# paritybit-ai/XFL

Measured on AMD Instinct MI355X. Metric: 2048-bit Paillier encrypts/s (device-resident), higher is better.
Workload: dtype u32; 1 GPU; DJN private-key (CRT) encrypt, obfuscated, precision 7, 1000000 float64 plaintexts/GPU resident in HBM; key_bits=2048, elements_per_gpu=1000000, fixed_base_window_bits=23, fixed_base_window_split=False, parallelism=shard1, table_bytes=193273528320

## Files before the change

### xfl_amd/csrc/keyconst.hpp

```cpp
#pragma once
#include <algorithm>
#include <cstdint>
#include <stdexcept>
#include <utility>
#include <vector>

#include "hostbn.hpp"
#include "keydev.hpp"
#include "rns_layout.hpp"

namespace xhe {

struct ModSpec {
  int S, W;
  int S4() const { return (S + 3) & ~3; }
  BigU R() const { return pow2((size_t)W * S); }
};

struct KeySpec {
  int K;
  bool priv, djn;
  ModSpec mp2, mp2L, mp2X;
  ModSpec mp;
  ModSpec mn2, mn2X;
// ... 205 lines not shown
using PairF = const uint2* KeyDev::*;
using ModF = ModDev KeyDev::*;
using IntF = int KeyDev::*;

struct Dst {
  RowF w = nullptr;
  PairF d = nullptr;
  ModF m = nullptr;
  const uint32_t* ModDev::*mw = nullptr;
  size_t* off = nullptr;
  Dst(RowF f) : w(f) {}
  Dst(PairF f) : d(f) {}
  Dst(ModF mod, const uint32_t* ModDev::*f) : m(mod), mw(f) {}
  Dst(size_t* o) : off(o) {}
};

struct KeyImage {
  std::vector<uint32_t> words;
  KeyDev kd{};
  int rand_bits = 0, rand_words = 0;
  size_t hM_n2 = 0, hM_p2[2] = {0, 0};
  std::vector<uint32_t> hinvM_p[2];

  void put(const std::vector<uint32_t>& v, Dst dst, size_t min_words = 0) {
    const size_t off = words.size();
    const size_t len = (std::max(v.size(), min_words) + 3) & ~(size_t)3;
    words.resize(off + len, 0u);
    std::copy(v.begin(), v.end(), words.begin() + off);
    if (dst.off) *dst.off = off;
    else binds.push_back({dst, off});
  }
  void put_limbs(const BigU& x, const ModSpec& s, Dst dst) { put(x.to_limbs(s.W, s.S), dst, s.S4()); }
  void put_words(const BigU& x, int nw, Dst dst) {
    std::vector<uint32_t> v(nw);
    x.to_words(v.data(), nw);
    put(v, dst);
  }
  void put_mod(const BigU& M, const ModSpec& s, ModF m, int npow = 0) {
    const BigU R1 = mod(s.R(), M), R2 = mulmod(R1, R1, M), R3 = mulmod(R2, R1, M);
    put_limbs(M, s, {m, &ModDev::N});
    put_limbs(R1, s, {m, &ModDev::R1});
    put_limbs(R2, s, {m, &ModDev::R2});
    put_limbs(R3, s, {m, &ModDev::R3});
    (kd.*m).n0inv = mont_ninv(M.word(0), s.W);
    if (npow <= 0) return;
    std::vector<uint32_t> rows((size_t)npow * s.S4(), 0u);
    BigU x = mod(BigU(1), M);
    for (int j = 0; j < npow; ++j) {
      const std::vector<uint32_t> l = x.to_limbs(s.W, s.S);
      std::copy(l.begin(), l.end(), rows.begin() + (size_t)j * s.S4());
      x = mulmod(x, R1, M);
    }
    put(rows, {m, &ModDev::Rpow});
  }

  KeyDev bind(const uint32_t* base) const {
    KeyDev r = kd;
    for (const Binding& b : binds) {
      const uint32_t* p = base + b.off;
      if (b.dst.w) r.*b.dst.w = p;
      else if (b.dst.d) r.*b.dst.d = reinterpret_cast<const uint2*>(p);
      else (r.*b.dst.m).*b.dst.mw = p;
    }
    return r;
  }

 private:
  struct Binding {
    Dst dst;
    size_t off;
  };
  std::vector<Binding> binds;
};

namespace pq {
constexpr ModF m2[2] = {&KeyDev::p2, &KeyDev::q2}, m2L[2] = {&KeyDev::p2L, &KeyDev::q2L},
               m2X[2] = {&KeyDev::p2X, &KeyDev::q2X}, m1[2] = {&KeyDev::p, &KeyDev::q},
               dm[2] = {&KeyDev::dp, &KeyDev::dq};
constexpr RowF nprime[2] = {&KeyDev::p2_nprime, &KeyDev::q2_nprime}, rns[2] = {&KeyDev::rns_p, &KeyDev::rns_q},
               nR2[2] = {&KeyDev::nR2_p2, &KeyDev::nR2_q2}, nR2L[2] = {&KeyDev::nR2_p2L, &KeyDev::nR2_q2L},
               nR[2] = {&KeyDev::nR_p2, &KeyDev::nR_q2}, R1C[2] = {&KeyDev::R1C_p2X, &KeyDev::R1C_q2X},
               nR2C[2] = {&KeyDev::nR2C_p2X, &KeyDev::nR2C_q2X}, m1_words[2] = {&KeyDev::pm1_words, &KeyDev::qm1_words},
               inv_lim[2] = {&KeyDev::pinv_lim, &KeyDev::qinv_lim}, hR[2] = {&KeyDev::hpR, &KeyDev::hqR},
               topc[2] = {&KeyDev::topc_p, &KeyDev::topc_q}, e_words[2] = {&KeyDev::ep_words, &KeyDev::eq_words},
               x_kn2[2] = {&KeyDev::x_kn2_p, &KeyDev::x_kn2_q}, x_rmn[2] = {&KeyDev::x_rmn_p, &KeyDev::x_rmn_q},
               x_topc[2] = {&KeyDev::x_topc_p, &KeyDev::x_topc_q}, x_fold[2] = {&KeyDev::x_fold_p, &KeyDev::x_fold_q},
               x_hpR[2] = {&KeyDev::x_hpR_p, &KeyDev::x_hpR_q};
constexpr PairF x_dwt[2] = {&KeyDev::x_dwt_p, &KeyDev::x_dwt_q}, x_dw[2] = {&KeyDev::x_dw_p, &KeyDev::x_dw_q};
constexpr IntF m1_bits[2] = {&KeyDev::pm1_bits, &KeyDev::qm1_bits}, e_bits[2] = {&KeyDev::ep_bits, &KeyDev::eq_bits};
}

struct Prime {
  BigU X, Y, X2, n, h;
};

struct DigitMod {
  const BigU& M;
  ModSpec s;
  BigU R, RM, Rinv;
  DigitMod(const BigU& M_, const ModSpec& s_) : M(M_), s(s_), R(s_.R()), RM(mod(R, M_)), Rinv(modinv(RM, M_)) {}
};

inline std::vector<uint32_t> digit_pairs(const DigitMod& d, const BigU& Xw) {
  const BigU e = mulmod(mod(Xw, d.M), d.Rinv, d.M);
  BigU Q;
  divmod(add(Xw, mul(d.R, sub(d.M, e))), d.M, &Q, nullptr);
  const BigU f = submod(mod(Q, d.M), d.RM, d.M);
  const std::vector<uint32_t> el = e.to_limbs(d.s.W, d.s.S), fl = f.to_limbs(d.s.W, d.s.S);
  std::vector<uint32_t> v(2 * (size_t)d.s.S);
  for (int i = 0; i < d.s.S; ++i) {
    v[2 * i] = el[i];
    v[2 * i + 1] = fl[i];
  }
  return v;
}

inline std::vector<uint32_t> mask_plus_e(const BigU& M, const BigU& RM, const ModSpec& s) {
  std::vector<uint32_t> v = submod(BigU(1), RM, M).to_limbs(s.W, s.S);
  for (auto& x : v) x += (1u << s.W) - 1u;
  return v;
}

inline void digit_modulus(KeyImage& im, const DigitMod& d, const BigU& M2, ModF m, RowF kn2, RowF rmn) {
  im.put_mod(d.M, d.s, m);
  BigU c;
  divmod(sub(add(d.R, d.M), BigU(1)), d.M, &c, nullptr);
  im.put_limbs(mul(c, M2), ModSpec{2 * d.s.S, d.s.W}, kn2);
  im.put_limbs(sub(d.R, d.M), d.s, rmn);
}

inline void n2_constants(KeyImage& im, const KeySpec& s, const BigU& n, const BigU& n2, const BigU* h_pub) {
  im.put_words(n, s.nw(), &KeyDev::n_words);
  im.put_words(n2, s.n2w(), &KeyDev::n2_words);
  BigU maxpos;
  divmod(n, BigU(3), &maxpos, nullptr);
  im.put_words(maxpos, s.nw(), &KeyDev::maxpos);
  im.put_words(sub(n, maxpos), s.nw(), &KeyDev::minneg);
  im.put_limbs(n, s.mp2, &KeyDev::n_lim);
  im.put_mod(n2, s.mn2, &KeyDev::n2, kRpowRows);
  im.put_mod(n2, s.mn2X, &KeyDev::n2X, kRpowRows);
  if (s.K == 2048) {
    BigU mu;
    divmod(pow2((size_t)s.bar.W * 2 * s.bar.S), n2, &mu, nullptr);
    im.put_limbs(mu, ModSpec{s.bar.S + 1, s.bar.W}, &KeyDev::n2_mu);
  }
  if (s.K == 2048) {
    const ModSpec& sw = s.wave;
    const BigU Rw = sw.R();
    im.put_limbs(n2, sw, &KeyDev::n2w_N);
    im.put_limbs(sub(Rw, modinv(n2, Rw)), sw, &KeyDev::n2w_np);
    const BigU Rwn = mod(Rw, n2), Rw2 = mulmod(Rwn, Rwn, n2);
    im.put_limbs(mulmod(Rw2, modinv(mod(s.mn2X.R(), n2), n2), n2), sw, &KeyDev::n2w_C);
    im.put_limbs(Rw2, sw, &KeyDev::n2w_R2);
  }
  im.put_mod(n, s.mp2L, &KeyDev::nL);
  im.put_limbs(n2, ModSpec{2 * s.mp2L.S, s.mp2L.W}, &KeyDev::n2_limL);
  const BigU Rn2 = mod(s.mn2.R(), n2);
  im.put_limbs(mulmod(n, mulmod(Rn2, Rn2, n2), n2), s.mn2, &KeyDev::nR2_n2);
  if (h_pub) im.put_limbs(mulmod(mod(*h_pub, n2), Rn2, n2), s.mn2, &im.hM_n2);
}

inline void ndigit_constants(KeyImage& im, const KeySpec& s, const BigU& n, const BigU& n2) {
  const DigitMod d(n, s.nd);
  digit_modulus(im, d, n2, &KeyDev::nd, &KeyDev::nd_kn2, &KeyDev::nd_rmn);
  const BigU Rn2 = mod(d.R, n2), R2 = mulmod(Rn2, Rn2, n2), R4 = mulmod(R2, R2, n2);
  im.put(digit_pairs(d, R2), &KeyDev::nd_d1);
  im.put(digit_pairs(d, R4), &KeyDev::nd_dw);
  im.put(digit_pairs(d, mulmod(R4, modinv(mod(s.mn2.R(), n2), n2), n2)), &KeyDev::nd_dwt);
  im.put(mask_plus_e(n, d.RM, d.s), &KeyDev::nd_topc);
}

inline void prime2_constants(KeyImage& im, const KeySpec& s, const Prime (&pr)[2], const BigU* h, int nwin) {
  const ModSpec &s2 = s.mp2, &sL = s.mp2L, &sx = s.mp2X;
  const BigU &p2 = pr[0].X2, &q2 = pr[1].X2;
  im.put_mod(p2, s2, &KeyDev::p2);
  for (int i = 0; i < 2; ++i) im.put_mod(pr[i].X2, sL, pq::m2L[i]);
  for (int i = 0; i < 2; ++i) im.put_mod(pr[i].X2, sx, pq::m2X[i]);
  im.put_mod(q2, s2, &KeyDev::q2);
  const BigU R = s2.R();
  if (s.K == 2048) {
    for (int i = 0; i < 2; ++i) im.put_limbs(sub(R, modinv(pr[i].X2, R)), s2, pq::nprime[i]);
    im.put(rnsh::bases().shared, &KeyDev::rns);
    for (int i = 0; i < 2; ++i) im.put(rnsh::prime_block(pr[i].X), pq::rns[i]);
  }
  const BigU Rm[2] = {mod(R, p2), mod(R, q2)};
  for (int i = 0; i < 2; ++i)
    im.put_limbs(mulmod(pr[i].n, mulmod(Rm[i], Rm[i], pr[i].X2), pr[i].X2), s2, pq::nR2[i]);
  const BigU RL = sL.R();
  for (int i = 0; i < 2; ++i) {
    const BigU RLm = mod(RL, pr[i].X2);
    im.put_limbs(mulmod(pr[i].n, mulmod(RLm, RLm, pr[i].X2), pr[i].X2), sL, pq::nR2L[i]);
  }
  for (int i = 0; i < 2; ++i) im.put_limbs(mulmod(pr[i].n, Rm[i], pr[i].X2), s2, pq::nR[i]);
  im.put_limbs(mulmod(modinv(q2, p2), Rm[0], p2), s2, &KeyDev::q2invR_p2);
  im.put_limbs(q2, s2, &KeyDev::q2_lim);
  im.put_limbs(shl(p2, 2), s2, &KeyDev::p2x4_lim);
  if (!s.djn) return;
  for (int i = 0; i < 2; ++i)
    im.put_limbs(mulmod(mod(*h, pr[i].X2), Rm[i], pr[i].X2), s2, &im.hM_p2[i]);
  const BigU Rx = sx.R(), Cexp = pow2((size_t)(sx.S - s2.S) * s2.W * nwin);
  for (int i = 0; i < 2; ++i) {
    const BigU& X2 = pr[i].X2;
    const BigU RxP = mod(Rx, X2), CR = mulmod(mod(Cexp, X2), RxP, X2);
    im.put_limbs(CR, sx, pq::R1C[i]);
    im.put_limbs(mulmod(pr[i].n, mulmod(CR, RxP, X2), X2), sx, pq::nR2C[i]);
  }
}

inline void decrypt_constants(KeyImage& im, const KeySpec& s, const BigU& n, Prime (&pr)[2]) {
  const ModSpec& s1 = s.mp;
  const BigU T = s1.R();
  for (int i = 0; i < 2; ++i) im.put_mod(pr[i].X, s1, pq::m1[i]);
  for (int i = 0; i < 2; ++i) {
    const BigU m1 = sub(pr[i].X, BigU(1));
    im.kd.*pq::m1_bits[i] = (int)m1.bits();
    im.put_words(m1, s.nw() / 2 + 1, pq::m1_words[i]);
  }
  for (int i = 0; i < 2; ++i) im.put_limbs(modinv(pr[i].X, T), s1, pq::inv_lim[i]);
  BigU Tm[2];
  for (int i = 0; i < 2; ++i) {
    const BigU& X = pr[i].X;
    const BigU x = mod(add(BigU(1), mul(sub(X, BigU(1)), n)), pr[i].X2);
    BigU L;
    divmod(sub(x, BigU(1)), X, &L, nullptr);
    pr[i].h = modinv(L, X);
    Tm[i] = mod(T, X);
  }
  for (int i = 0; i < 2; ++i) im.put_limbs(mulmod(pr[i].h, Tm[i], pr[i].X), s1, pq::hR[i]);
  im.put_limbs(mulmod(modinv(pr[1].X, pr[0].X), Tm[0], pr[0].X), s1, &KeyDev::qinvpR);
  im.put_limbs(pr[1].X, s1, &KeyDev::q_lim);
  if (s.K == 2048)
    for (int i = 0; i < 2; ++i) im.put(mask_plus_e(pr[i].X, mod(s.pmd.R(), pr[i].X), s.pmd), pq::topc[i]);
}

inline void pdigit_constants(KeyImage& im, const KeySpec& s, const Prime& pr, int i) {
  const BigU &X = pr.X, &X2 = pr.X2;
  const DigitMod d(X, s.pd);
  digit_modulus(im, d, X2, pq::dm[i], pq::x_kn2[i], pq::x_rmn[i]);
  im.put(mask_plus_e(X, d.RM, d.s), pq::x_topc[i]);
  im.put_limbs(mulmod(mod(pr.Y, X), mulmod(mulmod(d.RM, d.RM, X), d.RM, X), X), d.s, pq::x_fold[i]);
  const BigU Rx2 = mod(d.R, X2), R2 = mulmod(Rx2, Rx2, X2), R4 = mulmod(R2, R2, X2);
  im.put(digit_pairs(d, mulmod(R4, modinv(mod(s.mp2.R(), X2), X2), X2)), pq::x_dwt[i]);
  im.put(digit_pairs(d, R4), pq::x_dw[i]);
  im.put_limbs(mulmod(pr.h, d.RM, X), d.s, pq::x_hpR[i]);
}

inline void exponent_constants(KeyImage& im, const KeySpec& s, const BigU& n, const Prime (&pr)[2]) {
  im.put_limbs(shl(pr[0].X, 1), s.mp, &KeyDev::p2x_lim);
  im.put_limbs(pr[0].X, s.mp, &KeyDev::p_lim);
  for (int i = 0; i < 2; ++i) {
    const BigU e = mod(n, mul(pr[i].X, sub(pr[i].X, BigU(1))));
    im.kd.*pq::e_bits[i] = (int)e.bits();
    im.put_words(e, s.nw(), pq::e_words[i]);
  }
}

inline std::vector<uint32_t> inverse_base_limbs(const ModSpec& s, const BigU& h, const BigU& P) {
  std::vector<uint32_t> v = mulmod(modinv(mod(h, P), P), mod(s.R(), P), P).to_limbs(s.W, s.S);
  v.resize((size_t)s.S4(), 0u);
  return v;
}

inline KeyImage derive_key_constants(const KeySpec& s, const BigU& n, const BigU* p, const BigU* q, const BigU* h) {
  KeyImage im;
  KeyDev& kd = im.kd;
  kd.K = s.K;
  kd.nw = s.nw();
  kd.n2w = s.n2w();
  kd.priv = s.priv;
  kd.djn = s.djn;
  kd.n_bits = (int)n.bits();
  im.rand_bits = s.djn ? (int)(n.bits() / 2) : (int)n.bits();
  im.rand_words = (im.rand_bits + 31) / 32;
  if (s.djn) {
    kd.win = s.win;
    win_layout(im.rand_bits, s.win, s.priv && s.split, &kd.nwin, &kd.nhi);
  }
  const BigU n2 = mul(n, n);
  n2_constants(im, s, n, n2, s.djn && !s.priv ? h : nullptr);
  if (s.K == 2048) {
    kd.ndig = 1;
    ndigit_constants(im, s, n, n2);
  }
  if (!s.priv) return im;
  Prime pr[2] = {{*p, *q, mul(*p, *p), {}, {}}, {*q, *p, mul(*q, *q), {}, {}}};
  for (Prime& x : pr) x.n = mod(n, x.X2);
  prime2_constants(im, s, pr, h, kd.nwin);
  decrypt_constants(im, s, n, pr);
  if (s.K != 2048) {
    kd.pmdx_dec = 1;
    for (int i = 0; i < 2; ++i) pdigit_constants(im, s, pr[i], i);
  }
  exponent_constants(im, s, n, pr);
  if (s.K == 2048 && s.djn)
    for (int i = 0; i < 2; ++i) im.hinvM_p[i] = inverse_base_limbs(s.pmd, *h, pr[i].X);
  return im;
}

}
```

### xfl_amd/csrc/keydev.hpp

```cpp
#pragma once
#include <cstdint>

#include <hip/hip_vector_types.h>

namespace xhe {

struct ModDev {
  const uint32_t* N;
  const uint32_t* R1;
  const uint32_t* R2;
  const uint32_t* R3;
  uint32_t n0inv;
  const uint32_t* Rpow;
};

constexpr int kRawChunk = 32;
constexpr int kRpowRows = kRawChunk + 2;

struct KeyDev {
  int K, nw, n2w;
  int priv, djn;
  const uint32_t* n_words;
  const uint32_t* n2_words;
  const uint32_t* maxpos;
  const uint32_t* minneg;
  const uint32_t* n_lim;
  ModDev n2;
  const uint32_t* nR2_n2;
  const uint32_t* tab_n2;
  const uint32_t* ep_words;
  const uint32_t* eq_words;
  int ep_bits, eq_bits, n_bits;
  ModDev p2, q2;
  ModDev p2L, q2L;
  ModDev p2X, q2X;
  ModDev n2X;
  const uint32_t* nR2_p2;
  const uint32_t *nR_p2, *nR_q2;
  const uint32_t *nR2C_p2X, *nR2C_q2X;
  const uint32_t *R1C_p2X, *R1C_q2X;
  const uint32_t* nR2_q2;
  const uint32_t* nR2_p2L;
  const uint32_t* nR2_q2L;
  const uint32_t* q2invR_p2;
  const uint32_t* q2_lim;
  const uint32_t* p2x4_lim;
  const uint32_t* tab_p2;
  const uint32_t* tab_q2;
  int64_t tab_rs;
  int win, nwin, nhi;
  ModDev p, q;
  const uint32_t* pm1_words;
  const uint32_t* qm1_words;
  int pm1_bits, qm1_bits;
  const uint32_t* pinv_lim;
  const uint32_t* qinv_lim;
  const uint32_t* hpR;
  const uint32_t* hqR;
  const uint32_t* qinvpR;
  const uint32_t* q_lim;
  const uint32_t* p2x_lim;
  const uint32_t* p_lim;
  int pmd;
  const uint32_t *topc_p, *topc_q;
  int ndig;
  ModDev nd;
  const uint32_t *nd_kn2, *nd_rmn, *nd_topc;
  const uint2 *nd_dw, *nd_d1;
  const uint2* nd_dwt;
  int pub_nd;
  int pmdx;
  ModDev dp, dq;
  const uint32_t *x_kn2_p, *x_kn2_q, *x_rmn_p, *x_rmn_q, *x_topc_p, *x_topc_q, *x_fold_p, *x_fold_q;
  const uint2 *x_dwt_p, *x_dwt_q;
  int pmdx_dec;
  const uint2 *x_dw_p, *x_dw_q;
  const uint32_t *x_hpR_p, *x_hpR_q;
  const uint32_t *p2_nprime, *q2_nprime;
  const uint32_t *rns, *rns_p, *rns_q;
  const uint32_t *n2w_N, *n2w_np, *n2w_C, *n2w_R2;
  const uint32_t* n2_mu;
  ModDev nL;
  const uint32_t* n2_limL;
};

}
```

### xfl_amd/csrc/pdigit_dev.hpp

```cpp
#pragma once
#include "bn_dev.hpp"

namespace xhe {

struct PmdLdsQ {
  const uint32_t* q;
  XHE_DEV uint4 load4(int i) const { return *reinterpret_cast<const uint4*>(q + (i >> 2) * 256); }
};

template <int K_>
struct PMD {
  static constexpr int K = K_, W = 28, BL = 6;
  static constexpr int NQ = (2 * K + 3) / 4;
  static constexpr uint32_t MASK = (1u << W) - 1u;
  static_assert((K - 1) % BL == 0, "positions 1..K-1 in blocks of 6");
  static_assert((double)(3 * K + 2) * (double)(1ull << 57) < 18446744073709551616.0, "accumulator bound");

  uint32_t p[K];
  uint32_t n0inv;

  XHE_DEV void init(const uint32_t* __restrict__ P, uint32_t ninv) {
#pragma unroll
    for (int j = 0; j < K; ++j) p[j] = __builtin_amdgcn_readfirstlane(P[j]);
    n0inv = ninv;
// ... 191 lines not shown
      "v_mad_u64_u32 %10, vcc, %16, %33, %10\n\t"
      "v_mad_u64_u32 %11, vcc, %16, %34, %11"
        : "+v"(T1[j - 1]), "+v"(T1[j]), "+v"(T1[j + 1]), "+v"(T1[j + 2]), "+v"(T1[j + 3]), "+v"(T1[j + 4]),
          "+v"(T2[j - 1]), "+v"(T2[j]), "+v"(T2[j + 1]), "+v"(T2[j + 2]), "+v"(T2[j + 3]), "+v"(T2[j + 4])
        : "v"(T1[j + 5]), "v"(T2[j + 5]), "v"(e), "v"(m1), "v"(m2), "v"(a[j]), "v"(a[j + 1]), "v"(a[j + 2]),
          "v"(a[j + 3]), "v"(a[j + 4]), "v"(a[j + 5]), "v"(c[j]), "v"(c[j + 1]), "v"(c[j + 2]), "v"(c[j + 3]),
          "v"(c[j + 4]), "v"(c[j + 5]), "s"(p[j]), "s"(p[j + 1]), "s"(p[j + 2]), "s"(p[j + 3]), "s"(p[j + 4]),
          "s"(p[j + 5])
        : "vcc");
  }

  XHE_DEV void step_row(uint64_t (&T1)[K], uint64_t (&T2)[K], const uint32_t (&a)[K], const uint32_t (&c)[K],
                        uint32_t e, uint32_t en, uint32_t& m1, uint32_t& m2, uint64_t& x1, uint64_t& x2,
                        uint32_t topc) const {
    uint64_t x1n = 0, x2n = 0;
    uint32_t t1 = 0, t2 = 0, m1n = 0, m2n = 0;
    asm("v_mad_u64_u32 %0, vcc, %2, %4, %0\n\t"
        "v_mad_u64_u32 %1, vcc, %3, %4, %1"
        : "+v"(x1), "+v"(x2)
        : "v"(m1), "v"(m2), "s"(p[0])
        : "vcc");
#pragma unroll
    for (int b = 0; b < (K - 1) / BL; ++b) {
      const int j = 1 + BL * b;
      blk12_row(T1, T2, a, c, e, m1, m2, j);
      if (b == 0) {
        T1[0] += x1 >> W;
        T2[0] += x2 >> W;
        asm volatile("" : "+v"(T1[0]), "+v"(T2[0]));
      } else if (b == 1) {
        asm("v_mad_u64_u32 %0, vcc, %2, %3, %5\n\t"
            "v_mad_u64_u32 %1, vcc, %2, %4, %6"
            : "=&v"(x1n), "=&v"(x2n)
            : "v"(en), "v"(a[0]), "v"(c[0]), "v"(T1[0]), "v"(T2[0])
            : "vcc");
        asm volatile("" : "+v"(x1n), "+v"(x2n));
      } else if (b == 2) {
        t1 = (uint32_t)x1n * n0inv;
        t2 = (uint32_t)x2n * n0inv;
        asm volatile("" : "+v"(t1), "+v"(t2));
      } else if (b == 3) {
        m1n = t1 & MASK;
        m2n = t2 & MASK;
        asm volatile("" : "+v"(m1n), "+v"(m2n));
      }
      __builtin_amdgcn_sched_barrier(0);
    }
    T1[K - 1] = 0;
    T2[K - 1] = (uint64_t)(topc - m1);
    x1 = x1n;
    x2 = x2n;
    m1 = m1n;
    m2 = m2n;
  }

  XHE_DEV void mul_row(uint32_t (&a)[K], uint32_t (&c)[K], const uint32_t* slot, const uint32_t* topc) const {
    uint64_t T1[K], T2[K];
#pragma unroll
    for (int j = 0; j < K; ++j) T1[j] = T2[j] = 0;
    uint2 p0 = *reinterpret_cast<const uint2*>(slot);
    uint64_t x1 = mad64(p0.x, a[0], 0ull);
    uint64_t x2 = mad64(p0.x, c[0], 0ull);
    uint32_t m1 = ((uint32_t)x1 * n0inv) & MASK, m2 = ((uint32_t)x2 * n0inv) & MASK;
    for (int h = 0; h < K / 2; ++h) {
      const int k = 2 * h + 2;
      const uint2 tc = *reinterpret_cast<const uint2*>(topc + 2 * h);
      const uint2 p1 = *reinterpret_cast<const uint2*>(slot + (k >> 2) * 256 + (k & 2));
      __builtin_amdgcn_sched_barrier(0);
      step_row(T1, T2, a, c, p0.x, p0.y, m1, m2, x1, x2, tc.x);
      __builtin_amdgcn_sched_barrier(0);
      step_row(T1, T2, a, c, p0.y, p1.x, m1, m2, x1, x2, tc.y);
      __builtin_amdgcn_sched_barrier(0);
      p0 = p1;
    }
    if constexpr (K & 1) step_row(T1, T2, a, c, p0.x, 0u, m1, m2, x1, x2, topc[K - 1]);
    normalize(T1, a);
    normalize(T2, c);
  }

  static constexpr int EQ = (K + 3) / 4;
  static constexpr int LW = (W * K + 31) / 32;
  static_assert(EQ + (LW + 3) / 4 <= NQ, "e limbs and the log sum share the slot of an interleaved row");

  template <int HW, bool FIRST>
  XHE_DEV static void lam_add(uint32_t* slot, const uint32_t (&lam)[HW]) {
    constexpr int LQ = (LW + 3) / 4;
    static_assert(HW >= 1 && HW <= 4 * LQ, "at most a whole sum");
    uint32_t s[4 * LQ];
    if constexpr (FIRST) {
#pragma unroll
      for (int k = 0; k < 4 * LQ; ++k) s[k] = k < HW ? lam[k] : 0u;
    } else {
#pragma unroll
      for (int q = 0; q < LQ; ++q) {
        const uint4 v = *reinterpret_cast<const uint4*>(slot + (EQ + q) * 256);
        s[4 * q] = v.x, s[4 * q + 1] = v.y, s[4 * q + 2] = v.z, s[4 * q + 3] = v.w;
      }
      uint32_t cy = 0;
#pragma unroll
      for (int k = 0; k < LW; ++k) {
        const uint64_t x = (uint64_t)s[k] + (k < HW ? lam[k] : 0u) + cy;
        s[k] = (uint32_t)x;
        cy = (uint32_t)(x >> 32);
      }
    }
#pragma unroll
    for (int q = 0; q < LQ; ++q)
      *reinterpret_cast<uint4*>(slot + (EQ + q) * 256) = make_uint4(s[4 * q], s[4 * q + 1], s[4 * q + 2], s[4 * q + 3]);
  }
  XHE_DEV static void lam_add_slot(uint32_t* slot, const uint32_t* other) {
    constexpr int LQ = (LW + 3) / 4;
    uint32_t o[4 * LQ];
#pragma unroll
    for (int q = 0; q < LQ; ++q) {
      const uint4 v = *reinterpret_cast<const uint4*>(other + (EQ + q) * 256);
      o[4 * q] = v.x, o[4 * q + 1] = v.y, o[4 * q + 2] = v.z, o[4 * q + 3] = v.w;
    }
    lam_add<4 * LQ, false>(slot, o);
  }

  XHE_DEV void finish(const uint32_t (&a)[K], uint32_t (&c)[K], uint32_t* slot, const uint32_t* Pl) const {
    constexpr int LQ = (LW + 3) / 4;
    {
      uint32_t s[4 * LQ + 1];
#pragma unroll
      for (int q = 0; q < LQ; ++q) {
        const uint4 v = *reinterpret_cast<const uint4*>(slot + (EQ + q) * 256);
        s[4 * q] = v.x, s[4 * q + 1] = v.y, s[4 * q + 2] = v.z, s[4 * q + 3] = v.w;
      }
      s[4 * LQ] = 0u;
      auto limb = [&](int i) -> uint32_t {
        const int bit = W * i, k = bit >> 5, sh = bit & 31;
        return i < K ? (__builtin_amdgcn_alignbit(k + 1 < LW ? s[k + 1] : 0u, s[k], sh) & MASK) : 0u;
      };
#pragma unroll
      for (int q = 0; q < EQ; ++q)
        *reinterpret_cast<uint4*>(slot + q * 256) = make_uint4(limb(4 * q), limb(4 * q + 1), limb(4 * q + 2), limb(4 * q + 3));
    }
    __builtin_amdgcn_sched_barrier(0);
    uint32_t t[K];
#pragma unroll
    for (int j = 0; j < K; ++j) t[j] = a[j];
    Mont<K, W, 1> MN;
    MN.init(Pl, n0inv);
    MN.mul(t, PmdLdsQ{slot});
    uint32_t cy = 0;
#pragma unroll
    for (int j = 0; j < K; ++j) {
      const uint32_t x = c[j] + t[j] + cy;
      c[j] = j + 1 < K ? (x & MASK) : x;
      cy = j + 1 < K ? (x >> W) : 0u;
    }
  }

  XHE_DEV static void normalize(const uint64_t (&T)[K], uint32_t (&b)[K]) {
    uint64_t cy = 0;
#pragma unroll
    for (int j = 0; j < K; ++j) {
      const uint64_t x = T[j] + cy;
      b[j] = j + 1 < K ? ((uint32_t)x & MASK) : (uint32_t)x;
      cy = x >> W;
      __builtin_amdgcn_sched_barrier(0);
    }
  }

  XHE_DEV void to_mont2(const uint32_t (&a)[K], const uint32_t (&c)[K], uint32_t (&x)[2 * K]) const {
    uint64_t T[2 * K];
#pragma unroll
    for (int j = 0; j < K; ++j) {
      T[j] = 0;
      T[K + j] = a[j];
    }
#pragma unroll
    for (int i = 0; i < K; ++i) {
#pragma unroll
      for (int j = 0; j < K; ++j) T[i + j] = mad64s(c[j], p[i], T[i + j]);
    }
    uint64_t cy = 0;
#pragma unroll
    for (int j = 0; j < 2 * K; ++j) {
      const uint64_t v = T[j] + cy;
      x[j] = j + 1 < 2 * K ? ((uint32_t)v & MASK) : (uint32_t)v;
      cy = v >> W;
    }
  }
};

template <int K>
XHE_DEV void pmd_redc_wide(const PMD<K>& M, uint64_t (&T)[2 * K], uint32_t (&t)[K], uint32_t (&m)[K]) {
  constexpr uint32_t MASK = PMD<K>::MASK;
  uint64_t cy = 0;
#pragma unroll
  for (int i = 0; i < K; ++i) {
    uint64_t x = T[i] + cy;
    const uint32_t mi = ((uint32_t)x * M.n0inv) & MASK;
    m[i] = mi;
    x = mad64s(mi, M.p[0], x);
    cy = x >> 28;
#pragma unroll
    for (int j = 1; j < K; ++j) T[i + j] = mad64s(mi, M.p[j], T[i + j]);
    __builtin_amdgcn_sched_barrier(0);
  }
#pragma unroll
  for (int j = 0; j < K; ++j) {
    const uint64_t x = T[K + j] + cy;
    t[j] = j + 1 < K ? ((uint32_t)x & MASK) : (uint32_t)x;
    cy = x >> 28;
  }
}

template <int K>
XHE_DEV uint32_t pmd_sub(uint32_t (&r)[K], const uint32_t (&s)[K]) {
  int64_t br = 0;
#pragma unroll
  for (int j = 0; j < K; ++j) {
    const int64_t v = (int64_t)r[j] - (int64_t)s[j] + br;
    r[j] = (uint32_t)v & ((1u << 28) - 1u);
    br = v >> 28;
  }
  return br ? 1u : 0u;
}

template <int K>
XHE_DEV bool pmd_csub(const PMD<K>& M, uint32_t (&r)[K]) {
  int64_t br = 0;
#pragma unroll
  for (int j = 0; j < K; ++j) br = ((int64_t)r[j] - (int64_t)M.p[j] + br) >> 28;
  const bool ge = br == 0;
  br = 0;
#pragma unroll
  for (int j = 0; j < K; ++j) {
    const int64_t v = (int64_t)r[j] - (int64_t)(ge ? M.p[j] : 0u) + br;
    r[j] = (uint32_t)v & ((1u << 28) - 1u);
    br = v >> 28;
  }
  return ge;
}

template <int K>
XHE_DEV void pmd_mod_small(const PMD<K>& M, uint32_t (&m)[K]) {
  constexpr uint32_t MASK = PMD<K>::MASK;
  const uint32_t mt = (m[K - 1] << 4) | (m[K - 2] >> 24);
  const uint32_t pt = (M.p[K - 1] << 4) | (M.p[K - 2] >> 24);
  const uint32_t q = mt / (pt + 1u);
  uint64_t cy = 0;
  int64_t br = 0;
#pragma unroll
  for (int j = 0; j < K; ++j) {
    const uint64_t qp = (uint64_t)q * M.p[j] + cy;
    cy = qp >> 28;
    const int64_t v = (int64_t)m[j] - (int64_t)(qp & MASK) + br;
    m[j] = (uint32_t)v & MASK;
    br = v >> 28;
  }
#pragma unroll
  for (int t = 0; t < 3; ++t) pmd_csub<K>(M, m);
}

template <int K>
XHE_DEV void pmd_from_mont2(const PMD<K>& M, const uint32_t (&X)[2 * K], const uint32_t* RmodP, uint32_t (&e)[K],
                            uint32_t (&f)[K]) {
  uint32_t m[K];
  {
    uint64_t T[2 * K];
#pragma unroll
    for (int j = 0; j < 2 * K; ++j) T[j] = X[j];
    pmd_redc_wide<K>(M, T, e, m);
  }
  __builtin_amdgcn_sched_barrier(0);
  const bool ge = pmd_csub<K>(M, e);
  __builtin_amdgcn_sched_barrier(0);
  pmd_mod_small<K>(M, m);
  __builtin_amdgcn_sched_barrier(0);
  int64_t br = 0;
#pragma unroll
  for (int j = 0; j < K; ++j) {
    const int64_t v = (int64_t)(ge ? RmodP[j] : 0u) - (int64_t)m[j] + br;
    f[j] = (uint32_t)v & ((1u << 28) - 1u);
    br = v >> 28;
  }
  if (br) {
    int64_t cy = 0;
#pragma unroll
    for (int j = 0; j < K; ++j) {
      const int64_t v = (int64_t)f[j] + (int64_t)M.p[j] + cy;
      f[j] = (uint32_t)v & ((1u << 28) - 1u);
      cy = v >> 28;
    }
  }
}

// ... 648 lines not shown
```

### xfl_amd/csrc/xhe_kernels.hpp

```cpp
#pragma once
#include "bn_dev.hpp"
#include "keydev.hpp"
#include "pdigit_dev.hpp"

#include <type_traits>

namespace xhe {

enum : int32_t { ST_OK = 0, ST_OVERFLOW = 1, ST_VALUE = 2 };

struct EncVal {
  int32_t st, e;
  int neg, w;
  uint32_t v0, v1, v2;
};

XHE_DEV EncVal encode_value(double v, int mode, int e0, int has_max, int max_exp) {
  EncVal r{ST_OK, 0, 0, 0, 0u, 0u, 0u};
  uint64_t bits = __double_as_longlong(v);
  r.neg = (int)(bits >> 63);
  int bexp = (int)((bits >> 52) & 0x7FF);
  uint64_t frac = bits & ((1ull << 52) - 1);
  int e;
  if (mode == 0) {
// ... 415 lines not shown
                           uint32_t* __restrict__ ws) {
  constexpr int NQ = MP2::S4 / 4;
  MP2 M;
  M.init(Np, md.n0inv);
  uint32_t b[MP2::L];
  const uint32_t* ae = a_words + (size_t)e * aw;
  auto stage = [&](int w) XHE_INL {
    int64_t row0;
    const uint32_t d = win_digit(key, ae, aw, w, row0);
    const uint32_t* row = tab + (size_t)(row0 + d) * key.tab_rs;
#pragma unroll
    for (int k = 0; k < RW / 4; ++k)
      __builtin_amdgcn_global_load_lds((xhe_glb_void*)(row + 4 * k), (xhe_lds_void*)(img + k * 256), 16, 0, 0);
    asm volatile("s_waitcnt vmcnt(0)" ::: "memory");
    unpack_limbs_lds<MP2, RW>(img + (threadIdx.x & 63) * 4);
  };
  (void)nR2;
  stage(0);
#pragma unroll
  for (int k = 0; k < NQ; ++k) {
    const uint4 v = ALdsQ{mine}.load4(4 * k);
    if (4 * k < MP2::S) b[4 * k] = v.x;
    if (4 * k + 1 < MP2::S) b[4 * k + 1] = v.y;
    if (4 * k + 2 < MP2::S) b[4 * k + 2] = v.z;
    if (4 * k + 3 < MP2::S) b[4 * k + 3] = v.w;
  }
  for (int w = 1; w < key.nwin; ++w) {
    stage(w);
    M.mul(b, ALdsQ{mine});
  }
  SqLds<MP2>(img).put(b);
  M.load_words(b, m_words + (size_t)e * key.nw, key.nw);
  M.mul(b, ARow{nR});
  b[0] += 1u;
  M.mul(b, ALdsQ{mine});
  M.reduce_once(b);
  M.store_strided(b, ws + (size_t)prime * 2 * MP2::S4 * count + e, (int)count);
}

template <class MP2, int RW>
__global__ void __launch_bounds__(128, 2) k_djn_pow_lds(KeyDev key, const uint32_t* __restrict__ Np2,
                                                        const uint32_t* __restrict__ Nq2,
                                                        const uint32_t* __restrict__ m_words,
                                                        const uint32_t* __restrict__ a_words, int aw, int64_t count,
                                                        uint32_t* __restrict__ ws) {
  static_assert(MP2::TPI == 1, "LDS row staging is per lane");
  __shared__ __attribute__((aligned(16))) uint32_t img_all[2][(MP2::S4 / 4) * 256];
  const int64_t e = (int64_t)blockIdx.x * blockDim.x + threadIdx.x;
  const int prime = blockIdx.y;
  uint32_t* img = img_all[(threadIdx.x >> 6) & 1];
  if (e >= count) return;
  djn_prime_lds<MP2, RW>(key, prime ? Nq2 : Np2, prime ? key.q2 : key.p2, prime ? key.tab_q2 : key.tab_p2,
                     prime ? key.nR2_q2 : key.nR2_p2, prime ? key.nR_q2 : key.nR_p2, m_words, a_words, aw, count, e,
                     prime, img, img + (threadIdx.x & 63) * 4, ws);
}

template <class MP2, int KP, int RW, int G = 1>
__global__ void __launch_bounds__(128, 2) k_djn_pmd(KeyDev key, const uint32_t* __restrict__ Pp,
                                                    const uint32_t* __restrict__ Pq, const uint32_t* __restrict__ Np2,
                                                    const uint32_t* __restrict__ Nq2,
                                                    const uint32_t* __restrict__ m_words,
                                                    const uint32_t* __restrict__ a_words, int aw, int64_t count,
                                                    uint32_t* __restrict__ ws) {
  static_assert(MP2::TPI == 1 && MP2::S == 2 * KP && MP2::W == 28, "digits of the one-lane P^2 shape");
  using D = PMD<KP>;
  constexpr int NQ = D::NQ > MP2::S4 / 4 ? D::NQ : MP2::S4 / 4;
  __shared__ __attribute__((aligned(16))) uint32_t img_all[2][NQ * 256];
  __shared__ __attribute__((aligned(16))) uint32_t topc[(KP + 3) & ~3];
  const int prime = blockIdx.y;
  const uint32_t* tc = prime ? key.topc_q : key.topc_p;
  if (threadIdx.x < KP) topc[threadIdx.x] = tc[threadIdx.x];
  __syncthreads();
  static_assert(G >= 1 && G <= 64 && (G & (G - 1)) == 0, "lane groups of a power of two, inside one wave");
  const int64_t t = (int64_t)blockIdx.x * blockDim.x + threadIdx.x;
  const int64_t e = t / G;
  const int g = (int)(threadIdx.x & (G - 1));
  if (e >= count) return;
  uint32_t* img = img_all[(threadIdx.x >> 6) & 1];
  uint32_t* slot = img + (threadIdx.x & 63) * 4;
  const uint32_t* tab = prime ? key.tab_q2 : key.tab_p2;
  const uint32_t* ae = a_words + (size_t)e * aw;
  D M;
  M.init(prime ? Pq : Pp, prime ? key.q.n0inv : key.p.n0inv);
  auto stage = [&](int w, auto first) XHE_INL {
    int64_t row0;
    const uint32_t d = win_digit(key, ae, aw, w, row0);
    const uint32_t* row = tab + (size_t)(row0 + d) * key.tab_rs;
#pragma unroll
    for (int k = 0; k < RW / 8; ++k)
      __builtin_amdgcn_global_load_lds((xhe_glb_void*)(row + 4 * k), (xhe_lds_void*)(img + k * 256), 16, 0, 0);
    uint32_t lam[RW / 2];
#pragma unroll
    for (int k = 0; k < RW / 8; ++k) {
      const uint4 v = *reinterpret_cast<const uint4*>(row + RW / 2 + 4 * k);
      lam[4 * k] = v.x, lam[4 * k + 1] = v.y, lam[4 * k + 2] = v.z, lam[4 * k + 3] = v.w;
    }
    asm volatile("s_waitcnt vmcnt(0)" ::: "memory");
    D::template lam_add<RW / 2, decltype(first)::value>(slot, lam);
    unpack_e_lds<KP, RW / 2>(slot);
  };
  uint32_t a[KP], c[KP];
  if (G == 1 || g < key.nwin) {
    stage(g, std::true_type{});
#pragma unroll
    for (int q = 0; q < D::EQ; ++q) {
      const uint4 v = *reinterpret_cast<const uint4*>(slot + q * 256);
      if (4 * q < KP) a[4 * q] = v.x;
      if (4 * q + 1 < KP) a[4 * q + 1] = v.y;
      if (4 * q + 2 < KP) a[4 * q + 2] = v.z;
      if (4 * q + 3 < KP) a[4 * q + 3] = v.w;
    }
#pragma unroll
    for (int j = 0; j < KP; ++j) c[j] = 0u;
  }
  for (int w = g + G; w < key.nwin; w += G) {
    stage(w, std::false_type{});
    M.mul_row(a, c, slot, topc);
  }
  if constexpr (G > 1) {
#pragma unroll
    for (int s = 1; s < G; s <<= 1) {
      const bool writer = (g & (2 * s - 1)) == s && g < key.nwin;
      const bool reader = (g & (2 * s - 1)) == 0 && g + s < key.nwin;
      if (reader) D::lam_add_slot(slot, slot + 4 * s);
      wave_sync_mem_();
      if (writer) {
#pragma unroll
        for (int q = 0; q < D::NQ; ++q)
          *reinterpret_cast<uint4*>(slot + q * 256) =
              make_uint4(2 * q < KP ? a[2 * q] : 0u, 2 * q < KP ? c[2 * q] : 0u, 2 * q + 1 < KP ? a[2 * q + 1] : 0u,
                         2 * q + 1 < KP ? c[2 * q + 1] : 0u);
      }
      wave_sync_mem_();
      if (reader) M.mul(a, c, slot + 4 * s, topc);
      wave_sync_mem_();
    }
    if (g != 0) return;
  }
  M.finish(a, c, slot, prime ? Pq : Pp);
  __builtin_amdgcn_sched_barrier(0);
  {
    uint32_t x[2 * KP];
    M.to_mont2(a, c, x);
#pragma unroll
    for (int q = 0; q < MP2::S4 / 4; ++q)
      *reinterpret_cast<uint4*>(slot + q * 256) =
          make_uint4(4 * q < 2 * KP ? x[4 * q] : 0u, 4 * q + 1 < 2 * KP ? x[4 * q + 1] : 0u,
                     4 * q + 2 < 2 * KP ? x[4 * q + 2] : 0u, 4 * q + 3 < 2 * KP ? x[4 * q + 3] : 0u);
  }
  MP2 N;
  N.init(prime ? Nq2 : Np2, prime ? key.q2.n0inv : key.p2.n0inv);
  uint32_t b[MP2::L];
  N.load_words(b, m_words + (size_t)e * key.nw, key.nw);
  N.mul(b, ARow{prime ? key.nR_q2 : key.nR_p2});
  b[0] += 1u;
  N.mul(b, ALdsQ{slot});
  N.reduce_once(b);
  N.store_strided(b, ws + (size_t)prime * 2 * MP2::S4 * count + e, (int)count);
}

template <int KP>
XHE_DEV void pmd_pow_uniform(const PMD<KP>& M, uint32_t (&a)[KP], uint32_t (&c)[KP], const uint32_t* ex, int ebits,
                             uint4* __restrict__ tab_base, int lane, int G, uint32_t* slot, const uint32_t* topc) {
  constexpr int NQ = PMD<KP>::NQ;
#define tab (tab_base + opaque_i(lane))
  auto quad = [&](int q) -> uint4 {
    return make_uint4(2 * q < KP ? a[2 * q] : 0u, 2 * q < KP ? c[2 * q] : 0u, 2 * q + 1 < KP ? a[2 * q + 1] : 0u,
                      2 * q + 1 < KP ? c[2 * q + 1] : 0u);
  };
  auto put_slot = [&]() XHE_INL {
#pragma unroll
    for (int q = 0; q < NQ; ++q) *reinterpret_cast<uint4*>(slot + q * 256) = quad(q);
  };
  auto put_tab = [&](int t) XHE_INL {
#pragma unroll
    for (int q = 0; q < NQ; ++q) tab[((size_t)t * NQ + q) * G] = quad(q);
  };
  auto tab_to_slot = [&](int t) XHE_INL {
    uint4 v[NQ];
#pragma unroll
    for (int q = 0; q < NQ; ++q) v[q] = tab[((size_t)t * NQ + q) * G];
#pragma unroll
    for (int q = 0; q < NQ; ++q) *reinterpret_cast<uint4*>(slot + q * 256) = v[q];
  };
  auto tab_to_regs = [&](int t) XHE_INL {
#pragma unroll
    for (int q = 0; q < NQ; ++q) {
      const uint4 v = tab[((size_t)t * NQ + q) * G];
      if (2 * q < KP) a[2 * q] = v.x, c[2 * q] = v.y;
      if (2 * q + 1 < KP) a[2 * q + 1] = v.z, c[2 * q + 1] = v.w;
    }
  };
  auto bit = [&](int i) { return (ex[i >> 5] >> (i & 31)) & 1u; };
  int i = ebits - 1;
  while (i >= 0 && !bit(i)) --i;
  int pend_sq = 0, pend_mul = -1;
  bool sq = false;
  auto next_op = [&]() -> bool {
    while (true) {
      if (pend_sq > 0) {
        put_slot();
        --pend_sq;
        sq = true;
        return true;
      }
      if (pend_mul >= 0) {
        tab_to_slot(pend_mul);
        pend_mul = -1;
        sq = false;
        return true;
      }
      if (i < 0) return false;
      if (!bit(i)) {
        pend_sq = 1;
        --i;
      } else {
        int j = i - 4 < 0 ? 0 : i - 4;
        while (!bit(j)) ++j;
        uint32_t val = 0;
        for (int k = i; k >= j; --k) val = (val << 1) | bit(k);
        pend_sq = i - j + 1;
        pend_mul = (int)(val >> 1);
        i = j - 1;
      }
    }
  };
  put_tab(0);
  put_slot();
  sq = true;
  int t = -1;
#pragma unroll 1
  while (true) {
    if (sq) M.sqr(a, c, slot, topc);
    else M.mul(a, c, slot, topc);
    if (t < 15) {
      sq = false;
      if (t < 0) {
        put_slot();
        tab_to_regs(0);
      } else {
        put_tab(t + 1);
// ... 1781 lines not shown
```

Baseline: 46.23 million encrypts/s.

## Fold plaintext term into the log-sum instead of a mod-p² multiply at the end

The DJN CRT encrypt used to finish with a full mod-p² multiply by (1 + m·n). It now reduces the plaintext mod p with a wide REDC, multiplies it by a precomputed per-prime constant mu = Y·R^4 mod p, and writes the result into the log-sum slot before the window accumulation. With the (1 + λp)-style term folded into the accumulated sum, the final step becomes a single redc_wide against zero plus reduce_once, dropping two mod-p² multiplies and an LDS round trip. The output index is now recomputed from the block and thread IDs. This adds a small mod-p multiply per element and new key constants, and it relies on the algebra being exactly equivalent.

```diff
diff --git a/xfl_amd/csrc/keyconst.hpp b/xfl_amd/csrc/keyconst.hpp
--- a/xfl_amd/csrc/keyconst.hpp
+++ b/xfl_amd/csrc/keyconst.hpp
@@ -311,7 +311,8 @@
                nR[2] = {&KeyDev::nR_p2, &KeyDev::nR_q2}, R1C[2] = {&KeyDev::R1C_p2X, &KeyDev::R1C_q2X},
                nR2C[2] = {&KeyDev::nR2C_p2X, &KeyDev::nR2C_q2X}, m1_words[2] = {&KeyDev::pm1_words, &KeyDev::qm1_words},
                inv_lim[2] = {&KeyDev::pinv_lim, &KeyDev::qinv_lim}, hR[2] = {&KeyDev::hpR, &KeyDev::hqR},
-               topc[2] = {&KeyDev::topc_p, &KeyDev::topc_q}, e_words[2] = {&KeyDev::ep_words, &KeyDev::eq_words},
+               topc[2] = {&KeyDev::topc_p, &KeyDev::topc_q}, mu[2] = {&KeyDev::mu_p, &KeyDev::mu_q},
+               e_words[2] = {&KeyDev::ep_words, &KeyDev::eq_words},
                x_kn2[2] = {&KeyDev::x_kn2_p, &KeyDev::x_kn2_q}, x_rmn[2] = {&KeyDev::x_rmn_p, &KeyDev::x_rmn_q},
                x_topc[2] = {&KeyDev::x_topc_p, &KeyDev::x_topc_q}, x_fold[2] = {&KeyDev::x_fold_p, &KeyDev::x_fold_q},
                x_hpR[2] = {&KeyDev::x_hpR_p, &KeyDev::x_hpR_q};
@@ -460,6 +461,11 @@
   im.put_limbs(pr[1].X, s1, &KeyDev::q_lim);
   if (s.K == 2048)
     for (int i = 0; i < 2; ++i) im.put(mask_plus_e(pr[i].X, mod(s.pmd.R(), pr[i].X), s.pmd), pq::topc[i]);
+  if (s.K == 2048 && s.djn)
+    for (int i = 0; i < 2; ++i) {
+      const BigU &X = pr[i].X, RX = mod(s.pmd.R(), X), R2 = mulmod(RX, RX, X);
+      im.put_limbs(mulmod(mod(pr[i].Y, X), mulmod(R2, R2, X), X), s.pmd, pq::mu[i]);
+    }
 }
 
 inline void pdigit_constants(KeyImage& im, const KeySpec& s, const Prime& pr, int i) {
diff --git a/xfl_amd/csrc/keydev.hpp b/xfl_amd/csrc/keydev.hpp
--- a/xfl_amd/csrc/keydev.hpp
+++ b/xfl_amd/csrc/keydev.hpp
@@ -63,6 +63,7 @@
   const uint32_t* p_lim;
   int pmd;
   const uint32_t *topc_p, *topc_q;
+  const uint32_t *mu_p, *mu_q;
   int ndig;
   ModDev nd;
   const uint32_t *nd_kn2, *nd_rmn, *nd_topc;
diff --git a/xfl_amd/csrc/pdigit_dev.hpp b/xfl_amd/csrc/pdigit_dev.hpp
--- a/xfl_amd/csrc/pdigit_dev.hpp
+++ b/xfl_amd/csrc/pdigit_dev.hpp
@@ -297,27 +297,26 @@
   static constexpr int LW = (W * K + 31) / 32;
   static_assert(EQ + (LW + 3) / 4 <= NQ, "e limbs and the log sum share the slot of an interleaved row");
 
-  template <int HW, bool FIRST>
+  XHE_DEV static void lam_zero(uint32_t* slot) {
+#pragma unroll
+    for (int q = 0; q < (LW + 3) / 4; ++q) *reinterpret_cast<uint4*>(slot + (EQ + q) * 256) = make_uint4(0u, 0u, 0u, 0u);
+  }
+  template <int HW>
   XHE_DEV static void lam_add(uint32_t* slot, const uint32_t (&lam)[HW]) {
     constexpr int LQ = (LW + 3) / 4;
     static_assert(HW >= 1 && HW <= 4 * LQ, "at most a whole sum");
     uint32_t s[4 * LQ];
-    if constexpr (FIRST) {
-#pragma unroll
-      for (int k = 0; k < 4 * LQ; ++k) s[k] = k < HW ? lam[k] : 0u;
-    } else {
-#pragma unroll
-      for (int q = 0; q < LQ; ++q) {
-        const uint4 v = *reinterpret_cast<const uint4*>(slot + (EQ + q) * 256);
-        s[4 * q] = v.x, s[4 * q + 1] = v.y, s[4 * q + 2] = v.z, s[4 * q + 3] = v.w;
-      }
-      uint32_t cy = 0;
-#pragma unroll
-      for (int k = 0; k < LW; ++k) {
-        const uint64_t x = (uint64_t)s[k] + (k < HW ? lam[k] : 0u) + cy;
-        s[k] = (uint32_t)x;
-        cy = (uint32_t)(x >> 32);
-      }
+#pragma unroll
+    for (int q = 0; q < LQ; ++q) {
+      const uint4 v = *reinterpret_cast<const uint4*>(slot + (EQ + q) * 256);
+      s[4 * q] = v.x, s[4 * q + 1] = v.y, s[4 * q + 2] = v.z, s[4 * q + 3] = v.w;
+    }
+    uint32_t cy = 0;
+#pragma unroll
+    for (int k = 0; k < LW; ++k) {
+      const uint64_t x = (uint64_t)s[k] + (k < HW ? lam[k] : 0u) + cy;
+      s[k] = (uint32_t)x;
+      cy = (uint32_t)(x >> 32);
     }
 #pragma unroll
     for (int q = 0; q < LQ; ++q)
@@ -331,7 +330,7 @@
       const uint4 v = *reinterpret_cast<const uint4*>(other + (EQ + q) * 256);
       o[4 * q] = v.x, o[4 * q + 1] = v.y, o[4 * q + 2] = v.z, o[4 * q + 3] = v.w;
     }
-    lam_add<4 * LQ, false>(slot, o);
+    lam_add<4 * LQ>(slot, o);
   }
 
   XHE_DEV void finish(const uint32_t (&a)[K], uint32_t (&c)[K], uint32_t* slot, const uint32_t* Pl) const {
@@ -422,6 +421,42 @@
     t[j] = j + 1 < K ? ((uint32_t)x & MASK) : (uint32_t)x;
     cy = x >> 28;
   }
+}
+
+template <int K>
+XHE_DEV void pmd_lam_plain(const PMD<K>& M, uint32_t* slot, const uint32_t* __restrict__ mw, int nw,
+                           const uint32_t* mu, const uint32_t* Pl) {
+  using D = PMD<K>;
+  constexpr int LQ = (D::LW + 3) / 4;
+  uint32_t t[K];
+  {
+    uint64_t T[2 * K];
+#pragma unroll
+    for (int j = 0; j < 2 * K; ++j) {
+      const int bit = 28 * j, k = bit >> 5, sh = bit & 31;
+      const uint32_t lo = word_or0(mw, k, nw);
+      const uint32_t hi = sh + 28 > 32 ? word_or0(mw, k + 1, nw) : 0u;
+      T[j] = (uint32_t)((((uint64_t)hi << 32) | lo) >> sh) & D::MASK;
+    }
+    uint32_t q[K];
+    pmd_redc_wide<K>(M, T, t, q);
+  }
+  __builtin_amdgcn_sched_barrier(0);
+  Mont<K, 28, 1> MN;
+  MN.init(Pl, M.n0inv);
+  MN.mul(t, ARow{mu});
+  uint32_t s[4 * LQ];
+#pragma unroll
+  for (int k = 0; k < 4 * LQ; ++k) {
+    const int bit = 32 * k, j = bit / 28, sh = bit - 28 * j;
+    uint64_t v = j < K ? (uint64_t)t[j] : 0ull;
+    if (j + 1 < K) v |= (uint64_t)t[j + 1] << 28;
+    if (j + 2 < K) v |= (uint64_t)t[j + 2] << 56;
+    s[k] = k < D::LW ? (uint32_t)(v >> sh) : 0u;
+  }
+#pragma unroll
+  for (int q = 0; q < LQ; ++q)
+    *reinterpret_cast<uint4*>(slot + (D::EQ + q) * 256) = make_uint4(s[4 * q], s[4 * q + 1], s[4 * q + 2], s[4 * q + 3]);
 }
 
 template <int K>
diff --git a/xfl_amd/csrc/xhe_kernels.hpp b/xfl_amd/csrc/xhe_kernels.hpp
--- a/xfl_amd/csrc/xhe_kernels.hpp
+++ b/xfl_amd/csrc/xhe_kernels.hpp
@@ -521,7 +521,7 @@
   const uint32_t* ae = a_words + (size_t)e * aw;
   D M;
   M.init(prime ? Pq : Pp, prime ? key.q.n0inv : key.p.n0inv);
-  auto stage = [&](int w, auto first) XHE_INL {
+  auto stage = [&](int w) XHE_INL {
     int64_t row0;
     const uint32_t d = win_digit(key, ae, aw, w, row0);
     const uint32_t* row = tab + (size_t)(row0 + d) * key.tab_rs;
@@ -535,12 +535,17 @@
       lam[4 * k] = v.x, lam[4 * k + 1] = v.y, lam[4 * k + 2] = v.z, lam[4 * k + 3] = v.w;
     }
     asm volatile("s_waitcnt vmcnt(0)" ::: "memory");
-    D::template lam_add<RW / 2, decltype(first)::value>(slot, lam);
+    D::template lam_add<RW / 2>(slot, lam);
     unpack_e_lds<KP, RW / 2>(slot);
   };
+  if (G == 1 || g == 0)
+    pmd_lam_plain<KP>(M, slot, m_words + (size_t)e * key.nw, key.nw, prime ? key.mu_q : key.mu_p, prime ? Pq : Pp);
+  else
+    D::lam_zero(slot);
+  __builtin_amdgcn_sched_barrier(0);
   uint32_t a[KP], c[KP];
   if (G == 1 || g < key.nwin) {
-    stage(g, std::true_type{});
+    stage(g);
 #pragma unroll
     for (int q = 0; q < D::EQ; ++q) {
       const uint4 v = *reinterpret_cast<const uint4*>(slot + q * 256);
@@ -553,7 +558,7 @@
     for (int j = 0; j < KP; ++j) c[j] = 0u;
   }
   for (int w = g + G; w < key.nwin; w += G) {
-    stage(w, std::false_type{});
+    stage(w);
     M.mul_row(a, c, slot, topc);
   }
   if constexpr (G > 1) {
@@ -578,24 +583,15 @@
   }
   M.finish(a, c, slot, prime ? Pq : Pp);
   __builtin_amdgcn_sched_barrier(0);
-  {
-    uint32_t x[2 * KP];
-    M.to_mont2(a, c, x);
-#pragma unroll
-    for (int q = 0; q < MP2::S4 / 4; ++q)
-      *reinterpret_cast<uint4*>(slot + q * 256) =
-          make_uint4(4 * q < 2 * KP ? x[4 * q] : 0u, 4 * q + 1 < 2 * KP ? x[4 * q + 1] : 0u,
-                     4 * q + 2 < 2 * KP ? x[4 * q + 2] : 0u, 4 * q + 3 < 2 * KP ? x[4 * q + 3] : 0u);
-  }
+  uint32_t b[MP2::L];
+  M.to_mont2(a, c, b);
+  __builtin_amdgcn_sched_barrier(0);
   MP2 N;
   N.init(prime ? Nq2 : Np2, prime ? key.q2.n0inv : key.p2.n0inv);
-  uint32_t b[MP2::L];
-  N.load_words(b, m_words + (size_t)e * key.nw, key.nw);
-  N.mul(b, ARow{prime ? key.nR_q2 : key.nR_p2});
-  b[0] += 1u;
-  N.mul(b, ALdsQ{slot});
+  N.redc_wide(b, AZero{});
   N.reduce_once(b);
-  N.store_strided(b, ws + (size_t)prime * 2 * MP2::S4 * count + e, (int)count);
+  const int64_t eo = ((int64_t)blockIdx.x * blockDim.x + (uint32_t)opaque_i((int)threadIdx.x)) / G;
+  N.store_strided(b, ws + (size_t)prime * 2 * MP2::S4 * count + eo, (int)count);
 }
 
 template <int KP>
```

Result: faster. 47.86 million encrypts/s, median of 6 (+3.5%).
